# nilsbore/gp_compressor

Measured on AMD Instinct MI355X. Metric: patches/sec (compress+predict), higher is better.
Workload: dtype f64; 1 GPU; C2 room scan: 8192 patches x 256 pts per GPU, RBF + Gaussian noise, dense Cholesky fit + predictive mean on the 20x20 grid (m=400); patches_per_gpu=8192, points_per_patch=256, grid_points=400, parallelism=1 GPU, kernel=dense_mfma_w1

## Files before the change

gp_compressor_amd/csrc/dense_mfma_w1.hip:

```cpp
#include <cstdio>
#include <cstdlib>
#include <type_traits>

#include "gpc_device.h"
#include "dense_internal.h"
#include "mfma_tile.h"

#define W1_NPAD_MAX 512
#define W1_C 4
#define W1_NDT 10
#define W1_NT_OF(npad) ((npad) / 16)
#define W1_TRI_OF(npad) (W1_NT_OF(npad) * (W1_NT_OF(npad) + 1) / 2)
#define W1_TILE(i, j) (((size_t)(i) * (size_t)((i) + 1) / 2 + (size_t)(j)) * MF_IMG)
#define W1_PACK_OF(npad) ((npad) <= 256)
#define W1_LNV_OF(npad) (W1_PACK_OF(npad) ? W1_NT_OF(npad) / 2 : W1_NT_OF(npad))


struct W1Params {
    DenseArgs a;
    double c_exp;
    double pivot_tol;
    double cs, noise_u, sfp, a_out;
    double* ws;
    double* linvt;
    int export_factor;
    unsigned long long* stamps;
};
#define W1_NPH 12
#ifdef W1_STAMPS
#define W1_STAMP(ph)                                                                                                 \
    do {                                                                                                             \
        __builtin_amdgcn_sched_barrier(0);                                                                           \
        const unsigned long long t_now_ = __builtin_amdgcn_s_memtime();                                              \
        st_acc_[ph] += t_now_ - t_prev_;                                                                             \
        t_prev_ = t_now_;                                                                                            \
        __builtin_amdgcn_sched_barrier(0);                                                                           \
    } while (0)
#else
#define W1_STAMP(ph) do { } while (0)
#endif

#define W1_LDS_SYNC()                                                                                                \
    do {                                                                                                             \
        __builtin_amdgcn_fence(__ATOMIC_SEQ_CST, "wavefront");                                                       \
        __builtin_amdgcn_wave_barrier();                                                                             \
    } while (0)

template <int A, int B, typename F>
__device__ static __forceinline__ void w1_static_for(F&& f)
{
    if constexpr (A < B) {
        f(std::integral_constant<int, A>{});
        w1_static_for<A + 1, B>(f);
    }
}
__host__ __device__ constexpr int w1_stream_col(int q)
{
    int kk = 0;
    while ((kk + 1) * (kk + 2) / 2 <= q) ++kk;
    return kk;
}
__host__ __device__ constexpr int w1_pstream_pair(int q)
{
    int pp = 0;
    while (2 * (pp + 1) * (pp + 1) <= q) ++pp;
    return pp;
}
#define W1_BW 20

__device__ static __forceinline__ d4 w1_mfma4_neg(d4 a, d4 b, d4 acc)
{
#pragma unroll
    for (int s = 0; s < 4; ++s) acc = __builtin_amdgcn_mfma_f64_16x16x4f64(a[s], b[s], acc, 0, 0, 1);
    return acc;
}
__device__ static __forceinline__ d4 w1_trsm(d4 lv, d4 src)
{
    const d4 z4 = d4{0.0, 0.0, 0.0, 0.0};
    d4 D = __builtin_amdgcn_mfma_f64_16x16x4f64(lv[0], src[0], z4, 0, 0, 0);
    D = __builtin_amdgcn_mfma_f64_16x16x4f64(lv[1], src[1], D, 0, 0, 0);
    D = __builtin_amdgcn_mfma_f64_16x16x4f64(lv[2], src[2], D, 0, 0, 0);
    return __builtin_amdgcn_mfma_f64_16x16x4f64(lv[3], src[3], D, 0, 0, 0);
}

template <int MODE, int CNT, bool DIAG>
__device__ static __forceinline__ void w1_gram_row(d4 (&v)[W1_C], const double* px0, const double* px1, const double* T, double sf, bool scale_sf,
                                                   double cexp, double noise, bool dbl, int n, int r, int c0, int lr, int lg)
{
    const int pi = MF_TS * r + lr;
    const double xi0 = px0[pi], xi1 = px1[pi];
#pragma unroll
    for (int t = 0; t < CNT; ++t) {
#pragma unroll
        for (int q = 0; q < 4; ++q) {
            const int pj = MF_TS * (c0 + t) + lg + 4 * q;
            const double d0 = xi0 - px0[pj], d1 = xi1 - px1[pj];
            const double sq = __builtin_fma(d0, d0, d1 * d1);
            v[t][q] = MODE == 0 ? gpc_exp_neg(cexp * sq, T) : gpc_expm_poly<MODE == 1 ? 7 : 5>(sq);
        }
    }
    if (scale_sf) {
#pragma unroll
        for (int t = 0; t < CNT; ++t)
#pragma unroll
            for (int q = 0; q < 4; ++q) v[t][q] *= sf;
    }
    if constexpr (DIAG) {
#pragma unroll
        for (int q = 0; q < 4; ++q) {
            double d = v[CNT - 1][q] + noise;
            if (dbl) d += noise;
            v[CNT - 1][q] = (lr == lg + 4 * q) ? d : v[CNT - 1][q];
        }
    }
    if (MF_TS * (r + 1) > n || MF_TS * (c0 + CNT) > n) {
#pragma unroll
        for (int t = 0; t < CNT; ++t) {
#pragma unroll
            for (int q = 0; q < 4; ++q) {
                const int pj = MF_TS * (c0 + t) + lg + 4 * q;
                if (pi >= n || pj >= n) v[t][q] = (pi == pj) ? 1.0 : 0.0;
            }
        }
    }
}

template <int W1_NPAD>
__global__ __launch_bounds__(64, 2) void dense_w1_kernel(W1Params g)
{
    constexpr int W1_NT = W1_NT_OF(W1_NPAD), W1_TRI = W1_TRI_OF(W1_NPAD);
    __shared__ __attribute__((aligned(16))) double T[GPC_EXP_TABLE_SIZE];
    __shared__ __attribute__((aligned(16))) double px0[W1_NPAD], px1[W1_NPAD], zv[W1_NPAD];
    __shared__ __attribute__((aligned(16))) double rsbuf[32], wsc[32];
    __shared__ __attribute__((aligned(16))) double LinvC[W1_C * MF_IMG];
    constexpr bool W1_PACK = W1_PACK_OF(W1_NPAD);
    constexpr int W1_LNV = W1_LNV_OF(W1_NPAD);
    __shared__ __attribute__((aligned(16))) double dgl[W1_PACK ? W1_LNV * MF_TS : 2];

    const DenseArgs& A = g.a;
    int lane = threadIdx.x;
    int lr = lane & 15, lg = lane >> 4;
#define W1_FRESH_LANE()                                                                                              \
    do {                                                                                                             \
        lane = mf_opaque(lane);                                                                                      \
        lr = lane & 15;                                                                                              \
        lg = lane >> 4;                                                                                              \
    } while (0)
    const int m = A.m;
    const double sf = A.prm.sigmaf_sq, cexp = g.c_exp;
    const bool dbl = A.prm.ref_double_noise != 0;
    const int patch = blockIdx.x;
    double* Lt = g.ws + (size_t)patch * W1_TRI * MF_IMG;
    double* LinvTg = g.linvt + (size_t)patch * W1_LNV * MF_IMG;

    gpc_exp_table_init(T);
    {
        const int o = __builtin_amdgcn_readfirstlane(A.off[patch]);
        const int n = __builtin_amdgcn_readfirstlane(A.off[patch + 1]) - o;
        double* fs = A.f_star + (size_t)patch * m;
        __syncthreads();
        if (n <= 0 || n > W1_NPAD) {
            for (int p = lane; p < m; p += 64) fs[p] = (n == 0) ? 0.0 : __builtin_nan("");
            if (lane == 0 && A.status) A.status[patch] = (n == 0) ? GPC_STATUS_OK : GPC_STATUS_NAN;
            return;
        }
        const int nt = __builtin_amdgcn_readfirstlane((n + MF_TS - 1) / MF_TS);
#ifdef W1_STAMPS
        unsigned long long st_acc_[W1_NPH] = {};
        unsigned long long t_prev_ = __builtin_amdgcn_s_memtime();
#endif

        const double xo0 = A.x0[o], xo1 = A.x1[o];
        double qr0[W1_NPAD / 64], qr1[W1_NPAD / 64];
        double mn0 = xo0, mx0 = xo0, mn1 = xo1, mx1 = xo1;
#pragma unroll
        for (int u = 0; u < W1_NPAD / 64; ++u) {
            const int i = lane + 64 * u;
            const bool live = i < n;
            qr0[u] = live ? A.x0[o + i] : xo0;
            qr1[u] = live ? A.x1[o + i] : xo1;
            mn0 = __builtin_fmin(mn0, qr0[u]); mx0 = __builtin_fmax(mx0, qr0[u]);
            mn1 = __builtin_fmin(mn1, qr1[u]); mx1 = __builtin_fmax(mx1, qr1[u]);
            zv[i] = live ? A.y[o + i] : 0.0;
        }
#pragma unroll
        for (int o_ = 32; o_ > 0; o_ >>= 1) {
            mn0 = __builtin_fmin(mn0, __shfl_xor(mn0, o_, 64)); mx0 = __builtin_fmax(mx0, __shfl_xor(mx0, o_, 64));
            mn1 = __builtin_fmin(mn1, __shfl_xor(mn1, o_, 64)); mx1 = __builtin_fmax(mx1, __shfl_xor(mx1, o_, 64));
        }
        int mode_g, mode_p;
        {
            const bool nan_box = !((mx0 - mn0) + (mx1 - mn1) < __builtin_inf());
            const double rx = mx0 - mn0, ry = mx1 - mn1;
            const double tg = nan_box ? __builtin_inf() : -cexp * __builtin_fma(rx, rx, ry * ry);
            const double hb = 0.5 * A.grid_res;
            const double bx = hb + __builtin_fmax(__builtin_fabs(mn0), __builtin_fabs(mx0));
            const double by = hb + __builtin_fmax(__builtin_fabs(mn1), __builtin_fabs(mx1));
            const double bq = __builtin_fmax(bx, by);
            const double tp = nan_box ? __builtin_inf() : -cexp * (bq * bq);
            mode_g = __builtin_amdgcn_readfirstlane(tg <= GPC_EXP_TINY_MAX ? 2 : tg <= GPC_EXP_SMALL_MAX ? 1 : 0);
            mode_p = __builtin_amdgcn_readfirstlane(tp <= GPC_EXP_TINY_MAX ? 2 : tp <= GPC_EXP_SMALL_MAX ? 1 : 0);
            if (mode_g == 0) mode_p = 0;
        }
        const bool scaled = mode_g > 0;
        {
            const double cs = scaled ? g.cs : 1.0;
            const double co0 = scaled ? xo0 : 0.0, co1 = scaled ? xo1 : 0.0;
#pragma unroll
            for (int u = 0; u < W1_NPAD / 64; ++u) {
                const int i = lane + 64 * u;
                const bool live = i < n;
                px0[i] = live ? cs * (qr0[u] - co0) : 0.0;
                px1[i] = live ? cs * (qr1[u] - co1) : 0.0;
            }
        }
        const bool scale_sf = g.export_factor != 0;
        const double noise_u = g.noise_u, ptol = g.pivot_tol;
        W1_LDS_SYNC();
#define W1_GRAM_ROW(v, CNT, DIAG, r, c0)                                                                              \
    do {                                                                                                             \
        if (mode_g == 2) w1_gram_row<2, CNT, DIAG>(v, px0, px1, T, sf, scale_sf, cexp, noise_u, dbl, n, r, c0, lr, lg);   \
        else if (mode_g == 1) w1_gram_row<1, CNT, DIAG>(v, px0, px1, T, sf, scale_sf, cexp, noise_u, dbl, n, r, c0, lr, lg); \
        else w1_gram_row<0, CNT, DIAG>(v, px0, px1, T, sf, scale_sf, cexp, noise_u, dbl, n, r, c0, lr, lg);            \
    } while (0)

        auto bw_close = [&](auto HASW, auto REV, const int k, const d4 img, d4& pa) __attribute__((always_inline)) {
            constexpr bool has_w = decltype(HASW)::value, rev = decltype(REV)::value;
            d4 ub = d4{0.0, 0.0, 0.0, 0.0};
            if constexpr (has_w) {
                const double tot = mf_row_reduce4(pa, lr);
                if ((lr & 3) == 0) wsc[lg + 4 * (lr >> 2)] = tot;
                W1_LDS_SYNC();
            }
            if (lr == 0) {
#pragma unroll
                for (int q4 = 0; q4 < 4; ++q4) {
                    const int e = rev ? MF_TS - 1 - (lg + 4 * q4) : lg + 4 * q4;
                    ub[q4] = has_w ? zv[MF_TS * k + e] - wsc[e] : zv[MF_TS * k + e];
                }
            }
            const d4 al = w1_trsm(img, ub);
            W1_LDS_SYNC();
            if (lr == 0) {
#pragma unroll
                for (int r = 0; r < 4; ++r) zv[MF_TS * k + (rev ? MF_TS - 1 - (lg + 4 * r) : lg + 4 * r)] = al[r];
            }
            W1_LDS_SYNC();
            pa = d4{0.0, 0.0, 0.0, 0.0};
        };
        auto bw_step = [&](auto P, const d4 img, d4& pa) __attribute__((always_inline)) {
            constexpr int q = decltype(P)::value;
            constexpr int kk = w1_stream_col(q), t = q - kk * (kk + 1) / 2;
            if (kk < nt) {
                const int k = nt - 1 - kk;
                if constexpr (t < kk) {
                    const double a_ = zv[MF_TS * (k + 1 + t) + lr];
                    pa += img * a_;
                } else {
                    bw_close(std::bool_constant<(kk > 0)>{}, std::false_type{}, k, img, pa);
                }
            }
        };
        bool bad = false;
        W1_STAMP(0);
#define W1_BLOCK_ROW(bi, kb, nb)                                                                                     \
    do {                                                                                                             \
        if ((bi) < (nb)) {                                                                                           \
            d4 gv[W1_C];                                                                                             \
            W1_GRAM_ROW(gv, (bi) + 1, true, (kb) + (bi), (kb));                                                      \
            _Pragma("unroll") for (int bc = 0; bc <= (bi); ++bc) tacc[(bi) * ((bi) + 1) / 2 + bc] = gv[bc];           \
        } else {                                                                                                     \
            _Pragma("unroll") for (int bc = 0; bc <= (bi); ++bc) tacc[(bi) * ((bi) + 1) / 2 + bc] = d4{0.0, 0.0, 0.0, 0.0}; \
        }                                                                                                            \
    } while (0)
#define W1_BLOCK_INIT(kb, nb)                                                                                        \
    do {                                                                                                             \
        _Pragma("unroll") for (int i = 0; i < W1_C; ++i) part[i] = 0.0;                                              \
                                             \
        __builtin_amdgcn_sched_barrier(0);                                                                           \
        W1_BLOCK_ROW(3, kb, nb);                                                                                     \
        __builtin_amdgcn_sched_barrier(0);                                                                           \
        W1_BLOCK_ROW(2, kb, nb);                                                                                     \
        __builtin_amdgcn_sched_barrier(0);                                                                           \
        W1_BLOCK_ROW(1, kb, nb);                                                                                     \
        __builtin_amdgcn_sched_barrier(0);                                                                           \
        W1_BLOCK_ROW(0, kb, nb);                                                                                     \
        __builtin_amdgcn_sched_barrier(0);                                                                           \
    } while (0)
        W1_STAMP(1);
        for (int k = 0;; k += W1_C) {
            const int nc = min(W1_C, nt - k);
            const int kl = k - 1;
            const bool last_step = k + W1_C >= nt;
            W1_FRESH_LANE();
            const double* rrow[W1_C];
#pragma unroll
            for (int i = 0; i < W1_C; ++i) rrow[i] = Lt + W1_TILE(k + min(i, nc - 1), 0);
            d4 tacc[W1_NDT];
            double part[W1_C];
            d4 op[2][W1_C];
#pragma unroll
            for (int i = 0; i < W1_C; ++i) op[0][i] = op[1][i] = d4{0.0, 0.0, 0.0, 0.0};
            if (k > 0) {
#pragma unroll
                for (int i = 0; i < W1_C; ++i) op[0][i] = mf_img_load(rrow[i], lane);
            }
            W1_BLOCK_INIT(k, nc);
            for (int j = 0; j < k; j += 2) {
#pragma unroll
                for (int h = 0; h < 2; ++h) {
                    const int jn = min(j + h + 1, kl);
#pragma unroll
                    for (int i = 0; i < W1_C; ++i) op[h ^ 1][i] = mf_img_load(rrow[i] + (size_t)jn * MF_IMG, lane);
#pragma unroll
                    for (int d = 0; d < W1_NDT; ++d) {
                        const int bi = d >= 6 ? 3 : d >= 3 ? 2 : d >= 1 ? 1 : 0, bc = d - bi * (bi + 1) / 2;
                        if (bi < nc) tacc[d] = w1_mfma4_neg(op[h][bc], op[h][bi], tacc[d]);
                    }
                    const double* zq = zv + MF_TS * (j + h) + lg;
                    const double z0 = zq[0], z1 = zq[4], z2 = zq[8], z3 = zq[12];
#pragma unroll
                    for (int c = 0; c < W1_C; ++c) part[c] += (op[h][c][0] * z0 + op[h][c][1] * z1) + (op[h][c][2] * z2 + op[h][c][3] * z3);
                }
            }
            W1_STAMP(2);
            W1_FRESH_LANE();
            d4 Lb[W1_C * (W1_C - 1) / 2];
#pragma unroll
            for (int q = 0; q < W1_C * (W1_C - 1) / 2; ++q) Lb[q] = d4{0.0, 0.0, 0.0, 0.0};
            bool ok = mf_diag_factor_c(tacc[0], rsbuf, LinvC, W1_PACK ? nullptr : LinvTg + (size_t)k * MF_IMG, ptol, lane);
            W1_LDS_SYNC();
            if (g.export_factor) mf_img_store(Lt + W1_TILE(k, k), lane, mf_img_load(LinvC, lane));
#pragma unroll
            for (int i = 1; i < W1_C; ++i) {
                if (ok && i < nc) {
#pragma unroll
                    for (int c = 0; c < i; ++c) {
                        d4 Tt = tacc[i * (i + 1) / 2 + c];
#pragma unroll
                        for (int c2 = 0; c2 < c; ++c2) Tt = w1_mfma4_neg(Lb[c * (c - 1) / 2 + c2], Lb[i * (i - 1) / 2 + c2], Tt);
                        const d4 lvc = mf_img_load(LinvC + c * MF_IMG, mf_opaque(lane));
                        const d4 L = w1_trsm(lvc, Tt);
                        Lb[i * (i - 1) / 2 + c] = L;
                        mf_img_store(Lt + W1_TILE(k + i, k + c), lane, L);
                    }
                    d4 Dii = tacc[i * (i + 1) / 2 + i];
#pragma unroll
                    for (int c = 0; c < i; ++c) Dii = w1_mfma4_neg(Lb[i * (i - 1) / 2 + c], Lb[i * (i - 1) / 2 + c], Dii);
                    ok = mf_diag_factor_c(Dii, rsbuf, LinvC + i * MF_IMG, W1_PACK ? nullptr : LinvTg + (size_t)(k + i) * MF_IMG, ptol, lane);
                    W1_LDS_SYNC();
                    if (g.export_factor) mf_img_store(Lt + W1_TILE(k + i, k + i), lane, mf_img_load(LinvC + i * MF_IMG, mf_opaque(lane)));
                }
            }
            if (!ok) { bad = true; break; }
            if constexpr (W1_PACK) {
                if (!last_step) {
#pragma unroll
                    for (int h = 0; h < 2; ++h) {
                        const int lp = mf_opaque(lane), pr = (k >> 1) + h;
                        const double* Lo = LinvC + (2 * h + 1) * MF_IMG;
                        const d4 pk = mf_tri_pack(mf_img_load_t(LinvC + 2 * h * MF_IMG, lp), mf_img_load_tr(Lo, lp));
                        mf_img_store(LinvTg + (size_t)pr * MF_IMG, lp, pk);
                        if (lp < MF_TS) dgl[MF_TS * pr + lp] = Lo[mf_img_rc(MF_TS - 1 - lp, MF_TS - 1 - lp)];
                    }
                }
            }
            W1_STAMP(3);
            W1_FRESH_LANE();
#pragma unroll
            for (int c = 0; c < W1_C; ++c) {
                if (c < nc) {
                    const int pj = MF_TS * (k + c) + lr;
                    double pp = part[c];
#pragma unroll
                    for (int c2 = 0; c2 < c; ++c2) {
                        const d4 lb = Lb[c * (c - 1) / 2 + c2];
                        const double* zq = zv + MF_TS * (k + c2) + lg;
                        pp += (lb[0] * zq[0] + lb[1] * zq[4]) + (lb[2] * zq[8] + lb[3] * zq[12]);
                    }
                    pp += __shfl_xor(pp, 16, 64);
                    pp += __shfl_xor(pp, 32, 64);
                    const double yv = zv[pj];
                    W1_LDS_SYNC();
                    if (lg == 0) zv[pj] = yv - pp;
                    W1_LDS_SYNC();
                    const d4 lv = mf_img_load(LinvC + c * MF_IMG, mf_opaque(lane));
                    const double* tq = zv + MF_TS * (k + c) + lg;
                    double zz = (lv[0] * tq[0] + lv[1] * tq[4]) + (lv[2] * tq[8] + lv[3] * tq[12]);
                    zz += __shfl_xor(zz, 16, 64);
                    zz += __shfl_xor(zz, 32, 64);
                    W1_LDS_SYNC();
                    if (lg == 0) zv[pj] = zz;
                    W1_LDS_SYNC();
                }
            }
            W1_STAMP(4);
            const int rows_tot = nt - (k + nc);
            if (rows_tot == 0) {
                __syncthreads();
                break;
            }
            if (k > 0) __syncthreads();
            const int npass = (rows_tot + 3) / 4;
            const int klp = k - 1;
            if (k == 0) {
                for (int pi_ = 0; pi_ < npass; ++pi_) {
                    const int first_row0 = (pi_ + 1 < npass) ? 4 * (pi_ + 1) : 0;
                    const int np4 = min(4, rows_tot - first_row0);
                    W1_FRESH_LANE();
                    d4 cy[W1_C][4];
#pragma unroll
                    for (int t = 0; t < 4; ++t) {
                        const int r_ = W1_C + first_row0 + min(t, np4 - 1);
                        d4 gv[W1_C];
                        W1_GRAM_ROW(gv, 2, false, r_, 0);
                        cy[0][t] = gv[0]; cy[1][t] = gv[1];
                        __builtin_amdgcn_sched_barrier(0);
                        W1_GRAM_ROW(gv, 2, false, r_, 2);
                        cy[2][t] = gv[0]; cy[3][t] = gv[1];
                        __builtin_amdgcn_sched_barrier(0);
                    }
                    W1_STAMP(5);
#pragma unroll
                    for (int c = 0; c < W1_C; ++c) {
                        const d4 lv = mf_img_load(LinvC + c * MF_IMG, mf_opaque(lane));
#pragma unroll
                        for (int t = 0; t < 4; ++t) {
#pragma unroll
                            for (int c2 = 0; c2 < c; ++c2) cy[c][t] = w1_mfma4_neg(Lb[c * (c - 1) / 2 + c2], cy[c2][t], cy[c][t]);
                            cy[c][t] = w1_trsm(lv, cy[c][t]);
                            if (t < np4) mf_img_store(Lt + W1_TILE(W1_C + first_row0 + t, c), lane, cy[c][t]);
                        }
                    }
                    W1_STAMP(7);
                }
            }
            if (k > 0) {
                for (int pi_ = 0; pi_ < npass; ++pi_) {
                    const int first_row = (pi_ + 1 < npass) ? 4 * (pi_ + 1) : 0;
                    const int np4 = min(4, rows_tot - first_row);
                    W1_FRESH_LANE();
                    d4 cy[W1_C][4];
                    int rr[4];
                    const double* rw_[4];
#pragma unroll
                    for (int t = 0; t < 4; ++t) {
                        rr[t] = k + W1_C + first_row + min(t, np4 - 1);
                        rw_[t] = Lt + W1_TILE(rr[t], 0);
                    }
                    d4 A2[2][W1_C], B[4];
#pragma unroll
                    for (int c = 0; c < W1_C; ++c) A2[0][c] = mf_img_load(rrow[c], lane);
#pragma unroll
                    for (int t = 0; t < 4; ++t) B[t] = mf_img_load(rw_[t], lane);
#pragma unroll
                    for (int t = 0; t < 4; ++t) {
                        d4 gv[W1_C];
                        W1_GRAM_ROW(gv, 2, false, rr[t], k);
                        cy[0][t] = gv[0]; cy[1][t] = gv[1];
                        __builtin_amdgcn_sched_barrier(0);
                        W1_GRAM_ROW(gv, 2, false, rr[t], k + 2);
                        cy[2][t] = gv[0]; cy[3][t] = gv[1];
                        __builtin_amdgcn_sched_barrier(0);
                    }
                    W1_STAMP(5);
                    d4 Lq[W1_C * (W1_C - 1) / 2];
#define W1_PASS_J(st, jn, PREFETCH)                                                                                  \
    do {                                                                                                             \
                                      \
        if (PREFETCH) {                                                                                              \
            _Pragma("unroll") for (int c = 0; c < W1_C; ++c) A2[(st) ^ 1][c] = mf_img_load(rrow[c] + (size_t)(jn) * MF_IMG, lane); \
        }                                                                                                            \
        __builtin_amdgcn_sched_barrier(0);                                                                           \
        _Pragma("unroll") for (int t = 0; t < 4; ++t) {                                                              \
            _Pragma("unroll") for (int c = 0; c < W1_C; ++c) cy[c][t] = w1_mfma4_neg(A2[st][c], B[t], cy[c][t]);      \
            __builtin_amdgcn_sched_barrier(0);                                                                       \
            if (PREFETCH) B[t] = mf_img_load(rw_[t] + (size_t)(jn) * MF_IMG, lane);                                    \
            else {      \
                if (t < 3) Lq[t] = mf_img_load(Lt + W1_TILE(k + (t == 0 ? 1 : 2), k + (t == 2 ? 1 : 0)), lane);      \
                else {                                                                                               \
                    _Pragma("unroll") for (int c2 = 0; c2 < 3; ++c2) Lq[3 + c2] = mf_img_load(Lt + W1_TILE(k + 3, k + c2), lane); \
                }                                                                                                    \
            }                                                                                                        \
            __builtin_amdgcn_sched_barrier(0);                                                                       \
        }                                                                                                            \
    } while (0)
                    for (int j = 0; j + 2 < k; j += 2) {
                        W1_PASS_J(0, j + 1, true);
                        W1_PASS_J(1, j + 2, true);
                    }
                    W1_PASS_J(0, klp, true);
                    W1_PASS_J(1, klp, false);
#undef W1_PASS_J
                    W1_STAMP(6);
                    W1_FRESH_LANE();
#pragma unroll
                    for (int c = 0; c < W1_C; ++c) {
                        const d4 lv = mf_img_load(LinvC + c * MF_IMG, mf_opaque(lane));
#pragma unroll
                        for (int t = 0; t < 4; ++t) {
#pragma unroll
                            for (int c2 = 0; c2 < c; ++c2) cy[c][t] = w1_mfma4_neg(Lq[c * (c - 1) / 2 + c2], cy[c2][t], cy[c][t]);
                            cy[c][t] = w1_trsm(lv, cy[c][t]);
                            if (t < np4) mf_img_store(Lt + W1_TILE(rr[t], k + c), lane, cy[c][t]);
                        }
                    }
                    W1_STAMP(7);
                }
            }
            __syncthreads();
            W1_STAMP(8);
        }
#undef W1_BLOCK_INIT
#undef W1_BLOCK_ROW

        if (bad) {
            for (int p = lane; p < m; p += 64) fs[p] = __builtin_nan("");
            if (A.alpha_out)
                for (int i = lane; i < n; i += 64) A.alpha_out[o + i] = __builtin_nan("");
            if (lane == 0 && A.status) A.status[patch] = GPC_STATUS_NOT_SPD;
            return;
        }

        if constexpr (W1_PACK) {
            W1_FRESH_LANE();
            constexpr int NP = W1_NT;
            constexpr int SLEN = NP * NP / 2;
            const int nte = (nt + 1) & ~1, kls = (nt - 1) & ~(W1_C - 1);
            d4 win[W1_BW];
            auto stream_addr = [&](auto P) __attribute__((always_inline)) -> const double* {
                constexpr int q = decltype(P)::value;
                constexpr int pp = w1_pstream_pair(q), i = q - 2 * pp * pp;
                if constexpr (i == 2 * pp) {
                    const int k = nte - 1 - 2 * pp;
                    return (k >= 1 && k - 1 < kls) ? LinvTg + (size_t)(k >> 1) * MF_IMG : Lt;
                } else {
                    constexpr int kk = i < 2 * pp ? 2 * pp : 2 * pp + 1, t = i < 2 * pp ? i : i - 2 * pp - 1;
                    const int k = nte - 1 - kk, kq = max(k, 0);
                    return (k >= 0 && k + 1 + t < nt) ? Lt + W1_TILE(kq + 1 + t, kq) : Lt;
                }
            };
            w1_static_for<0, W1_BW>([&](auto P) __attribute__((always_inline)) {
                constexpr int q = decltype(P)::value;
                win[q] = mf_img_load_nt(stream_addr(P), lane);
            });
            d4 pa = d4{0.0, 0.0, 0.0, 0.0};
            double* const held = LinvC + (W1_C - 1) * MF_IMG;
            w1_static_for<0, SLEN>([&](auto P) __attribute__((always_inline)) {
                constexpr int q = decltype(P)::value;
                constexpr int pp = w1_pstream_pair(q), i = q - 2 * pp * pp;
                const d4 img = win[q % W1_BW];
                if constexpr (i == 2 * pp) {
                    const int k = nte - 1 - 2 * pp;
                    if (k >= 1) {
                        d4 lo;
                        bool in_lds = false;
                        if constexpr (pp < W1_C / 2) in_lds = k - 1 >= kls;
                        if (in_lds) {
                            const double* Lc = LinvC + (k - 1 - kls) * MF_IMG;
                            lo = mf_img_load_tr(Lc + MF_IMG, lane);
                        } else {
                            mf_img_store(held, lane, mf_tri_upper(img));
                            lo = mf_tri_lower(img, dgl[MF_TS * (k >> 1) + lr]);
                            W1_LDS_SYNC();
                        }
                        if (k < nt) bw_close(std::bool_constant<(pp > 0)>{}, std::true_type{}, k, lo, pa);
                    }
                } else {
                    constexpr int kk = i < 2 * pp ? 2 * pp : 2 * pp + 1, t = i < 2 * pp ? i : i - 2 * pp - 1;
                    const int k = nte - 1 - kk;
                    if (k >= 0 && k + 1 + t < nt) {
                        const double a_ = zv[MF_TS * (k + 1 + t) + lr];
                        pa += img * a_;
                    }
                    if constexpr (i == 4 * pp + 1) {
                        if (k >= 0) {
                            bool in_lds = false;
                            if constexpr (pp < W1_C / 2) in_lds = k >= kls;
                            const d4 up = in_lds ? mf_img_load_t(LinvC + (k - kls) * MF_IMG, lane) : mf_img_load(held, lane);
                            bw_close(std::true_type{}, std::false_type{}, k, up, pa);
                        }
                    }
                }
                if constexpr (q + W1_BW < SLEN) {
                    win[q % W1_BW] = mf_img_load_nt(stream_addr(std::integral_constant<int, q + W1_BW>{}), lane);
                }
            });
        } else {
            W1_FRESH_LANE();
            constexpr int NP = W1_NPAD / MF_TS;
            constexpr int SLEN = NP * (NP + 1) / 2;
            d4 win[W1_BW];
            auto stream_addr = [&](auto P) __attribute__((always_inline)) -> const double* {
                constexpr int q = decltype(P)::value;
                constexpr int kk = w1_stream_col(q), t = q - kk * (kk + 1) / 2;
                const int kq = max(nt - 1 - kk, 0);
                const double* ad = (t < kk) ? Lt + W1_TILE(kq + 1 + t, kq) : LinvTg + (size_t)kq * MF_IMG;
                return kk < nt ? ad : Lt;
            };
            w1_static_for<0, W1_BW>([&](auto P) __attribute__((always_inline)) {
                constexpr int q = decltype(P)::value;
                win[q] = mf_img_load_nt(stream_addr(P), lane);
            });
            d4 pa = d4{0.0, 0.0, 0.0, 0.0};
            w1_static_for<0, SLEN>([&](auto P) __attribute__((always_inline)) {
                constexpr int q = decltype(P)::value;
                bw_step(P, win[q % W1_BW], pa);
                if constexpr (q + W1_BW < SLEN) {
                    win[q % W1_BW] = mf_img_load_nt(stream_addr(std::integral_constant<int, q + W1_BW>{}), lane);
                }
            });
        }
        W1_STAMP(9);
        double* av = zv;
        if (A.alpha_out)
            for (int i = lane; i < n; i += 64) A.alpha_out[o + i] = av[i] * g.a_out;

        W1_FRESH_LANE();
        if (m <= 0) {
        } else if (A.xs0 == nullptr && A.grid_sz <= 32) {
            const int sz = A.grid_sz;
            const double res = A.grid_res;
            d4 P[2][2];
#pragma unroll
            for (int mt = 0; mt < 2; ++mt)
#pragma unroll
                for (int nl = 0; nl < 2; ++nl) P[mt][nl] = d4{0.0, 0.0, 0.0, 0.0};
            double gqx[2], gqy[2];
            const double cs = scaled ? g.cs : 1.0, co0 = scaled ? A.x0[o] : 0.0, co1 = scaled ? A.x1[o] : 0.0;
            const double argc = scaled ? -1.0 : cexp, sfp = g.sfp;
#pragma unroll
            for (int h = 0; h < 2; ++h) {
                const double gq = res * (((double)(16 * h + lr) + 0.5) / (double)sz - 0.5);
                gqx[h] = cs * (gq - co0);
                gqy[h] = cs * (gq - co1);
            }
            auto predict_loop = [&](auto mode_tag) __attribute__((always_inline)) {
                constexpr int MP = decltype(mode_tag)::value;
                for (int ibase = 0; ibase < n; ibase += 32) {
#pragma unroll
                    for (int s = 0; s < 8; ++s) {
                        const int i = ibase + 4 * s + lg;
                        const int ic = min(i, W1_NPAD - 1);
                        const double al = (i < n) ? sfp * av[ic] : 0.0;
                        const double xi0 = px0[ic], xi1 = px1[ic];
                        double ea[2], eb[2];
#pragma unroll
                        for (int h = 0; h < 2; ++h) {
                            const double dy = gqy[h] - xi1, dx = gqx[h] - xi0;
                            if constexpr (MP == 0) {
                                ea[h] = gpc_exp_neg(argc * (dy * dy), T);
                                eb[h] = gpc_exp_neg(argc * (dx * dx), T) * al;
                            } else {
                                ea[h] = gpc_expm_poly<MP == 1 ? 7 : 5>(dy * dy);
                                eb[h] = gpc_expm_poly<MP == 1 ? 7 : 5>(dx * dx) * al;
                            }
                        }
#pragma unroll
                        for (int nl = 0; nl < 2; ++nl)
#pragma unroll
                            for (int mt = 0; mt < 2; ++mt)
                                P[mt][nl] = __builtin_amdgcn_mfma_f64_16x16x4f64(ea[mt], eb[nl], P[mt][nl], 0, 0, 0);
                    }
                }
            };
            if (mode_p == 2) predict_loop(std::integral_constant<int, 2>{});
            else if (mode_p == 1) predict_loop(std::integral_constant<int, 1>{});
            else predict_loop(std::integral_constant<int, 0>{});
#pragma unroll
            for (int mt = 0; mt < 2; ++mt)
#pragma unroll
                for (int nl = 0; nl < 2; ++nl)
#pragma unroll
                    for (int r = 0; r < 4; ++r) {
                        const int py = 16 * mt + lg + 4 * r, pxx = 16 * nl + lr;
                        if (py < sz && pxx < sz) fs[py * sz + pxx] = P[mt][nl][r];
                    }
        } else {
            const double cs = scaled ? g.cs : 1.0, co0 = scaled ? A.x0[o] : 0.0, co1 = scaled ? A.x1[o] : 0.0;
            const double argc = scaled ? -1.0 : cexp, sfp = g.sfp;
            for (int p = lane; p < m; p += 64) {
                double q0, q1;
                if (A.xs0) {
                    q0 = A.xs0[p];
                    q1 = A.xs1[p];
                } else {
                    const int gx = p % A.grid_sz, gy = p / A.grid_sz;
                    q0 = A.grid_res * (((double)gx + 0.5) / (double)A.grid_sz - 0.5);
                    q1 = A.grid_res * (((double)gy + 0.5) / (double)A.grid_sz - 0.5);
                }
                q0 = cs * (q0 - co0);
                q1 = cs * (q1 - co1);
                double s_ = 0.0;
                for (int i = 0; i < n; ++i) {
                    const double d0 = px0[i] - q0, d1 = px1[i] - q1;
                    s_ += gpc_exp_neg(argc * __builtin_fma(d0, d0, d1 * d1), T) * av[i];
                }
                fs[p] = sfp * s_;
            }
        }
        if (lane == 0 && A.status) A.status[patch] = GPC_STATUS_OK;
#ifdef W1_STAMPS
        W1_STAMP(10);
        if (g.stamps && lane == 0)
            for (int q_ = 0; q_ < W1_NPH; ++q_) atomicAdd(g.stamps + q_, st_acc_[q_]);
#endif
    }
}

static int w1_npad(const DenseArgs& a) { return a.n_max <= 256 ? 256 : W1_NPAD_MAX; }

bool dense_w1_supported(const DenseArgs& a)
{
    if (a.v_star) return a.n_max <= 256 && a.ny == 1 && !a.sel && a.xs0 != nullptr;
    return a.n_max <= W1_NPAD_MAX && a.ny == 1 && !a.sel;
}

#define W1_MAX_SLOTS 8192
static int w1_chunk(const DenseArgs& a, int cap_in)
{
    const char* e = getenv("GPC_W1_SLOTS");
    int cap = e && atoi(e) > 0 ? atoi(e) : W1_MAX_SLOTS;
    if (cap_in > 0 && cap_in < cap) cap = cap_in;
    return a.P < cap ? a.P : cap;
}

size_t dense_w1_ws_bytes(const gpc_ctx* ctx, const DenseArgs& a, int* grid_out, int cap)
{
    (void)ctx;
    const int grid = w1_chunk(a, cap);
    if (grid_out) *grid_out = grid;
    const int npad = w1_npad(a);
    return sizeof(double) * ((size_t)(W1_TRI_OF(npad) + W1_LNV_OF(npad)) * MF_IMG * (size_t)grid + (a.v_star ? (size_t)a.n_total : 0));
}

int dense_w1_launch(gpc_ctx* ctx, const DenseSite& site, const DenseArgs& a_in, int grid)
{
    DenseArgs a = a_in;
    double* v_star = a.v_star;
    a.v_star = nullptr;
    W1Params g;
    g.c_exp = (double)(-0.5f) / a.prm.l_sq;
    g.ws = reinterpret_cast<double*>(dense_ws(ctx, site));
    const int npad = w1_npad(a);
    g.linvt = g.ws + (size_t)W1_TRI_OF(npad) * MF_IMG * (size_t)grid;
    g.export_factor = v_star ? 1 : 0;
    const double sf = a.prm.sigmaf_sq;
    const bool unit = !v_star;
    g.cs = sqrt(-g.c_exp);
    g.noise_u = unit ? a.prm.noise / sf : a.prm.noise;
    g.pivot_tol = GPC_PIVOT_RTOL * (unit ? 1.0 + a.prm.noise / sf : sf + a.prm.noise);
    g.sfp = unit ? 1.0 : sf;
    g.a_out = unit ? 1.0 / sf : 1.0;
    g.stamps = nullptr;
    if (v_star) {
        a.m = 0;
        if (!a.alpha_out) a.alpha_out = g.linvt + (size_t)W1_LNV_OF(npad) * MF_IMG * (size_t)grid;
    }
    ctx->last_dense_kernel = v_star ? "dense_mfma_w1 + dense_variance" : npad == 256 ? "dense_mfma_w1" : "dense_mfma_w1_512";
#ifdef W1_STAMPS
    if (getenv("GPC_W1_STAMPS")) {
        GPC_HIP(ctx, hipMalloc(&g.stamps, sizeof(unsigned long long) * W1_NPH));
        GPC_HIP(ctx, hipMemsetAsync(g.stamps, 0, sizeof(unsigned long long) * W1_NPH, site.stream));
    }
#endif
    for (int base = 0; base < a.P; base += grid) {
        const int cnt = a.P - base < grid ? a.P - base : grid;
        g.a = a;
        g.a.P = cnt;
        g.a.off = a.off + base;
        g.a.f_star = a.f_star ? a.f_star + (size_t)base * a.ny * a_in.m : nullptr;
        g.a.status = a.status ? a.status + base : nullptr;
        if (npad == 256) hipLaunchKernelGGL((dense_w1_kernel<256>), dim3(cnt), dim3(64), 0, site.stream, g);
        else hipLaunchKernelGGL((dense_w1_kernel<W1_NPAD_MAX>), dim3(cnt), dim3(64), 0, site.stream, g);
        GPC_HIP(ctx, hipGetLastError());
        if (v_star) {
            DenseArgs av = g.a;
            av.m = a_in.m;
            const int rc = dense_variance_launch(ctx, site, av, W1_NT_OF(256), g.ws, a.alpha_out, v_star + (size_t)base * a_in.m);
            if (rc != GPC_OK) return rc;
        }
    }
#ifdef W1_STAMPS
    if (g.stamps) {
        unsigned long long h[W1_NPH];
        GPC_HIP(ctx, hipStreamSynchronize(site.stream));
        GPC_HIP(ctx, hipMemcpy(h, g.stamps, sizeof(h), hipMemcpyDeviceToHost));
        (void)hipFree(g.stamps);
        static const char* names[W1_NPH] = {"load", "sweep gram", "sweep loop", "chain", "forward", "pass gram", "pass loop", "pass trsm",
                                            "step fence", "backward", "predict", ""};
        unsigned long long tot = 0;
        for (int q = 0; q < W1_NPH; ++q) tot += h[q];
        fprintf(stderr, "[GPC_W1_STAMPS] mean s_memtime ticks per patch (total %.0f)\n", (double)tot / a.P);
        for (int q = 0; q < 11; ++q) fprintf(stderr, "  %-12s %9.0f  %5.1f %%\n", names[q], (double)h[q] / a.P, 100.0 * h[q] / tot);
    }
#endif
    return GPC_OK;
}
```

gp_compressor_amd/csrc/mfma_tile.h:

```cpp
#pragma once

#include "gpc_device.h"

typedef double d4 __attribute__((ext_vector_type(4)));
#define MF_TS 16

__device__ static __forceinline__ int mf_opaque(int v)
{
    asm volatile("" : "+v"(v));
    return v;
}

__device__ static __forceinline__ bool mf_wait_ge(unsigned lds_byte_addr, int k)
{
    int v, cnt;
    asm volatile(
        "s_mov_b32 %1, 0x100000\n\t"
        "1:\n\t"
        "ds_read_b32 %0, %2\n\t"
        "s_waitcnt lgkmcnt(0)\n\t"
        "v_cmp_gt_i32 vcc, %3, %0\n\t"
        "s_cbranch_vccz 2f\n\t"
        "s_sub_u32 %1, %1, 1\n\t"
        "s_cmp_eq_u32 %1, 0\n\t"
        "s_cbranch_scc1 2f\n\t"
        "s_sleep 1\n\t"
        "s_branch 1b\n\t"
        "2:\n\t"
        : "=&v"(v), "=&s"(cnt)
        : "v"(lds_byte_addr), "v"(k)
        : "vcc", "scc", "memory");
    return cnt != 0;
}
__device__ static __forceinline__ void mf_publish(int* word, int k)
{
    __hip_atomic_store(word, k, __ATOMIC_RELEASE, __HIP_MEMORY_SCOPE_WORKGROUP);
}

__device__ static __forceinline__ double mf_readlane(double v, int lane_const)
{
    const int lo = __builtin_amdgcn_readlane(__double2loint(v), lane_const);
    const int hi = __builtin_amdgcn_readlane(__double2hiint(v), lane_const);
    return __hiloint2double(hi, lo);
}

__device__ static __forceinline__ double mf_rsqrt(double d)
{
    double y = __builtin_amdgcn_rsq(d);
    double e = __builtin_fma(-d * y, y, 1.0);
    y = __builtin_fma(y * 0.5, e, y);
    e = __builtin_fma(-d * y, y, 1.0);
    y = __builtin_fma(y * 0.5, e, y);
    return y;
}
__device__ static __forceinline__ double mf_rcp(double d)
{
    double y = __builtin_amdgcn_rcp(d);
    double e = __builtin_fma(-d, y, 1.0);
    y = __builtin_fma(y, e, y);
    e = __builtin_fma(-d, y, 1.0);
    y = __builtin_fma(y, e, y);
    return y;
}

typedef double d2 __attribute__((ext_vector_type(2)));
#define MF_IMG 256
__device__ static __forceinline__ int mf_img_off(int l, int s) { return (s >> 1) * 128 + l * 2 + (s & 1); }
__device__ static __forceinline__ int mf_img_rc(int r, int c) { return mf_img_off(r + 16 * (c & 3), c >> 2); }
__device__ static __forceinline__ d4 mf_img_load(const double* img, int l)
{
    const d2 a = *reinterpret_cast<const d2*>(img + l * 2);
    const d2 b = *reinterpret_cast<const d2*>(img + 128 + l * 2);
    return d4{a[0], a[1], b[0], b[1]};
}
__device__ static __forceinline__ void mf_img_store(double* img, int l, d4 v)
{
    *reinterpret_cast<d2*>(img + l * 2) = d2{v[0], v[1]};
    *reinterpret_cast<d2*>(img + 128 + l * 2) = d2{v[2], v[3]};
}

__device__ static __forceinline__ d4 mf_img_load_nt(const double* img, int l)
{
    const d2 a = __builtin_nontemporal_load(reinterpret_cast<const d2*>(img + l * 2));
    const d2 b = __builtin_nontemporal_load(reinterpret_cast<const d2*>(img + 128 + l * 2));
    return d4{a[0], a[1], b[0], b[1]};
}
__device__ static __forceinline__ void mf_img_store_nt(double* img, int l, d4 v)
{
    __builtin_nontemporal_store(d2{v[0], v[1]}, reinterpret_cast<d2*>(img + l * 2));
    __builtin_nontemporal_store(d2{v[2], v[3]}, reinterpret_cast<d2*>(img + 128 + l * 2));
}

template <bool OPAQUE = false>
__device__ __forceinline__ static bool mf_diag_factor(d4 W, double* rsbuf, double* Linv_out, double* LinvT_out, double pivot_tol, int lane_in = -1)
{
    const int lane = OPAQUE ? mf_opaque(lane_in >= 0 ? lane_in : (int)(threadIdx.x & 63)) : (int)(threadIdx.x & 63);
    const int lr = lane & 15, lg = lane >> 4;
    double rp = mf_rcp(mf_readlane(W[0], 0));
    double rpv = (lg == 0 && lr > 0) ? rp : 0.0;
    double one_q = (lg == 0) ? 1.0 : 0.0, ev = (lane == 0) ? 1.0 : 0.0;
#pragma unroll
    for (int c = 0; c < MF_TS - 1; ++c) {
        const int q = c & 3, r = c >> 2, q1 = (c + 1) & 3, r1 = (c + 1) >> 2;
        if constexpr (!OPAQUE) {
            one_q = (lg == q) ? 1.0 : 0.0;
            ev = (lg == q && lr == c) ? 1.0 : 0.0;
        }
        const double a_op = W[r] * rpv;
        const double b_op = __builtin_fma(W[r], one_q, ev);
        const d4 Wn = __builtin_amdgcn_mfma_f64_16x16x4f64(a_op, b_op, W, 0, 0, 1);
        __builtin_amdgcn_sched_barrier(0);
        const double s01 = mf_readlane(W[r], 16 * q + c + 1);
        const double s11 = mf_readlane(W[r1], 16 * q1 + c + 1);
        const double t = s01 * rp;
        rp = mf_rcp(__builtin_fma(-t, s01, s11));
        if constexpr (OPAQUE) {
            const int lo_ = mf_opaque(lane);
            const int lr_ = lo_ & 15, lg_ = lo_ >> 4;
            rpv = (lg_ == q1 && lr_ > c + 1) ? rp : 0.0;
            one_q = (lg_ == q1) ? 1.0 : 0.0;
            ev = (lo_ == 16 * q1 + c + 1) ? 1.0 : 0.0;
        } else {
            rpv = (lg == q1 && lr > c + 1) ? rp : 0.0;
        }
        __builtin_amdgcn_sched_barrier(0);
        W = Wn;
    }
    const int lt_ = OPAQUE ? mf_opaque(lane) : lane;
    const int lrt = lt_ & 15, lgt = lt_ >> 4;
    const int rsel = lrt >> 2;
    const double pd = rsel == 0 ? W[0] : rsel == 1 ? W[1] : rsel == 2 ? W[2] : W[3];
    const bool on_diag = (lrt & 3) == lgt;
    const bool ok = __builtin_amdgcn_ballot_w64(on_diag && !(pd > pivot_tol)) == 0;
    const double rs = mf_rsqrt(on_diag ? pd : 1.0);
    if (on_diag) rsbuf[lrt] = rs;
    d4 fin;
#pragma unroll
    for (int r = 0; r < 4; ++r) {
        const int row = lgt + 4 * r;
        const double rsr = rsbuf[row];
        fin[r] = (lrt < row) ? W[r] * rsr : (lrt == row ? rsr : 0.0);
    }
    mf_img_store(LinvT_out, lt_, fin);
#pragma unroll
    for (int r = 0; r < 4; ++r) Linv_out[mf_img_rc(lgt + 4 * r, lrt)] = fin[r];
    return ok;
}

__device__ static __forceinline__ int mf_sel32(int v, unsigned long long mask)
{
    int r;
    asm("v_cndmask_b32_e64 %0, 0, %1, %2" : "=v"(r) : "v"(v), "s"(mask));
    return r;
}
__device__ static __forceinline__ double mf_sel64(double v, unsigned long long mask)
{
    return __hiloint2double(mf_sel32(__double2hiint(v), mask), mf_sel32(__double2loint(v), mask));
}
__device__ static __forceinline__ double mf_one_in(unsigned long long mask, int one_hi)
{
    return __hiloint2double(mf_sel32(one_hi, mask), 0);
}
__device__ __forceinline__ static bool mf_diag_factor_c(d4 W, double* rsbuf, double* Linv_out, double* LinvT_out, double pivot_tol, int lane_in)
{
    const int one_hi = 0x3FF00000;
    double rp = mf_rcp(mf_readlane(W[0], 0));
    double rpv = mf_sel64(rp, 0xFFFEull);
    double one_q = mf_one_in(0xFFFFull, one_hi);
    double ev = mf_one_in(0x1ull, one_hi);
#pragma unroll
    for (int c = 0; c < MF_TS - 1; ++c) {
        const int q = c & 3, r = c >> 2, q1 = (c + 1) & 3, r1 = (c + 1) >> 2;
        const double a_op = W[r] * rpv;
        const double b_op = __builtin_fma(W[r], one_q, ev);
        const d4 Wn = __builtin_amdgcn_mfma_f64_16x16x4f64(a_op, b_op, W, 0, 0, 1);
        __builtin_amdgcn_sched_barrier(0);
        const double s01 = mf_readlane(W[r], 16 * q + c + 1);
        const double s11 = mf_readlane(W[r1], 16 * q1 + c + 1);
        const double t = s01 * rp;
        rp = mf_rcp(__builtin_fma(-t, s01, s11));
        const unsigned long long slot = 0xFFFFull << (16 * q1);
        const unsigned long long below = ((0xFFFFull << (c + 2)) & 0xFFFFull) << (16 * q1);
        rpv = mf_sel64(rp, below);
        one_q = mf_one_in(slot, one_hi);
        ev = mf_one_in(1ull << (16 * q1 + c + 1), one_hi);
        __builtin_amdgcn_sched_barrier(0);
        W = Wn;
    }
    const int lt_ = mf_opaque(lane_in);
    const int lrt = lt_ & 15, lgt = lt_ >> 4;
    const int rsel = lrt >> 2;
    const double pd = rsel == 0 ? W[0] : rsel == 1 ? W[1] : rsel == 2 ? W[2] : W[3];
    const bool on_diag = (lrt & 3) == lgt;
    const bool ok = __builtin_amdgcn_ballot_w64(on_diag && !(pd > pivot_tol)) == 0;
    const double rs = mf_rsqrt(on_diag ? pd : 1.0);
    if (on_diag) rsbuf[lrt] = rs;
    d4 fin;
#pragma unroll
    for (int r = 0; r < 4; ++r) {
        const int row = lgt + 4 * r;
        const double rsr = rsbuf[row];
        fin[r] = (lrt < row) ? W[r] * rsr : (lrt == row ? rsr : 0.0);
    }
    if (LinvT_out) mf_img_store(LinvT_out, lt_, fin);
#pragma unroll
    for (int r = 0; r < 4; ++r) Linv_out[mf_img_rc(lgt + 4 * r, lrt)] = fin[r];
    return ok;
}

__host__ __device__ constexpr unsigned long long mf_tri_mask(int s, int kind)
{
    unsigned long long m = 0;
    for (int l = 0; l < 64; ++l) {
        const int r = l & 15, c = (l >> 4) + 4 * s;
        if (kind == 0 ? r <= c : kind == 1 ? r == c : r > c) m |= 1ull << l;
    }
    return m;
}
__device__ static __forceinline__ int mf_mix32(int a, int b, unsigned long long mask)
{
    int r;
    asm("v_cndmask_b32_e64 %0, %1, %2, %3" : "=v"(r) : "v"(b), "v"(a), "s"(mask));
    return r;
}
__device__ static __forceinline__ double mf_mix64(double a, double b, unsigned long long mask)
{
    return __hiloint2double(mf_mix32(__double2hiint(a), __double2hiint(b), mask), mf_mix32(__double2loint(a), __double2loint(b), mask));
}
__device__ static __forceinline__ d4 mf_tri_pack(d4 up, d4 lo)
{
    constexpr unsigned long long u0 = mf_tri_mask(0, 0), u1 = mf_tri_mask(1, 0), u2 = mf_tri_mask(2, 0), u3 = mf_tri_mask(3, 0);
    return d4{mf_mix64(up[0], lo[0], u0), mf_mix64(up[1], lo[1], u1), mf_mix64(up[2], lo[2], u2), mf_mix64(up[3], lo[3], u3)};
}
__device__ static __forceinline__ d4 mf_tri_upper(d4 p)
{
    constexpr unsigned long long u0 = mf_tri_mask(0, 0), u1 = mf_tri_mask(1, 0), u2 = mf_tri_mask(2, 0), u3 = mf_tri_mask(3, 0);
    return d4{mf_sel64(p[0], u0), mf_sel64(p[1], u1), mf_sel64(p[2], u2), mf_sel64(p[3], u3)};
}
__device__ static __forceinline__ d4 mf_tri_lower(d4 p, double dg)
{
    constexpr unsigned long long l0 = mf_tri_mask(0, 2), l1 = mf_tri_mask(1, 2), l2 = mf_tri_mask(2, 2), l3 = mf_tri_mask(3, 2);
    constexpr unsigned long long e0 = mf_tri_mask(0, 1), e1 = mf_tri_mask(1, 1), e2 = mf_tri_mask(2, 1), e3 = mf_tri_mask(3, 1);
    return d4{mf_mix64(dg, mf_sel64(p[0], l0), e0), mf_mix64(dg, mf_sel64(p[1], l1), e1), mf_mix64(dg, mf_sel64(p[2], l2), e2),
              mf_mix64(dg, mf_sel64(p[3], l3), e3)};
}
__device__ static __forceinline__ d4 mf_img_load_t(const double* img, int l)
{
    const int lr = l & 15, lg = l >> 4;
    return d4{img[mf_img_rc(lg, lr)], img[mf_img_rc(lg + 4, lr)], img[mf_img_rc(lg + 8, lr)], img[mf_img_rc(lg + 12, lr)]};
}
__device__ static __forceinline__ d4 mf_img_load_tr(const double* img, int l)
{
    const int lr = 15 - (l & 15), lg = 15 - (l >> 4);
    return d4{img[mf_img_rc(lg, lr)], img[mf_img_rc(lg - 4, lr)], img[mf_img_rc(lg - 8, lr)], img[mf_img_rc(lg - 12, lr)]};
}

__device__ static __forceinline__ double mf_row_dot(const double* img, int mr, const double* v)
{
    double s_ = 0.0;
#pragma unroll
    for (int gq = 0; gq < 4; ++gq) {
        const d4 ch = mf_img_load(img, mr + 16 * gq);
#pragma unroll
        for (int s = 0; s < 4; ++s) s_ = __builtin_fma(ch[s], v[gq + 4 * s], s_);
    }
    return s_;
}

template <int CTRL>
__device__ static __forceinline__ double mf_dpp(double v)
{
    const int lo = __builtin_amdgcn_mov_dpp(__double2loint(v), CTRL, 0xf, 0xf, true);
    const int hi = __builtin_amdgcn_mov_dpp(__double2hiint(v), CTRL, 0xf, 0xf, true);
    return __hiloint2double(hi, lo);
}
__device__ static __forceinline__ double mf_row_allsum(double v)
{
    v += mf_dpp<0x121>(v);
    v += mf_dpp<0x122>(v);
    v += mf_dpp<0x124>(v);
    v += mf_dpp<0x128>(v);
    return v;
}

__device__ static __forceinline__ double mf_row_reduce4(d4 x, int lr)
{
    const bool hi8 = (lr & 8) != 0, hi4 = (lr & 4) != 0;
    double k0 = hi8 ? x[2] : x[0], k1 = hi8 ? x[3] : x[1];
    const double s0 = hi8 ? x[0] : x[2], s1 = hi8 ? x[1] : x[3];
    k0 += mf_dpp<0x128>(s0);
    k1 += mf_dpp<0x128>(s1);
    double k = hi4 ? k1 : k0;
    const double sd = hi4 ? k0 : k1;
    k += mf_dpp<0x141>(sd);
    k += mf_dpp<0xB1>(k);
    k += mf_dpp<0x4E>(k);
    return k;
}
```

Baseline: 5.624 million patches/s.

## Reverse panel traversal order for cache reuse and pin select masks in SGPRs

The Cholesky panel update loop now walks prior tile columns from most recent to oldest, and the trailing-row update passes alternate between ascending and descending j order. This serpentine traversal is meant to reuse factor tiles still resident in cache from the previous pass. Select and mix masks are also materialised through explicit s_mov_b32 literals so the compiler keeps them in scalar registers instead of rematerialising them. The reordering changes the floating-point summation order of the accumulation, and the volatile asm may constrain scheduling.

Measured after the change: 5.608 million patches/s. No clear change (-0.3%).

```diff
diff --git a/gp_compressor_amd/csrc/dense_mfma_w1.hip b/gp_compressor_amd/csrc/dense_mfma_w1.hip
--- a/gp_compressor_amd/csrc/dense_mfma_w1.hip
+++ b/gp_compressor_amd/csrc/dense_mfma_w1.hip
@@ -303,13 +303,14 @@
             for (int i = 0; i < W1_C; ++i) op[0][i] = op[1][i] = d4{0.0, 0.0, 0.0, 0.0};
             if (k > 0) {
 #pragma unroll
-                for (int i = 0; i < W1_C; ++i) op[0][i] = mf_img_load(rrow[i], lane);
+                for (int i = 0; i < W1_C; ++i) op[0][i] = mf_img_load(rrow[i] + (size_t)kl * MF_IMG, lane);
             }
             W1_BLOCK_INIT(k, nc);
             for (int j = 0; j < k; j += 2) {
 #pragma unroll
                 for (int h = 0; h < 2; ++h) {
-                    const int jn = min(j + h + 1, kl);
+                    const int jc = kl - (j + h);
+                    const int jn = max(jc - 1, 0);
 #pragma unroll
                     for (int i = 0; i < W1_C; ++i) op[h ^ 1][i] = mf_img_load(rrow[i] + (size_t)jn * MF_IMG, lane);
 #pragma unroll
@@ -317,7 +318,7 @@
                         const int bi = d >= 6 ? 3 : d >= 3 ? 2 : d >= 1 ? 1 : 0, bc = d - bi * (bi + 1) / 2;
                         if (bi < nc) tacc[d] = w1_mfma4_neg(op[h][bc], op[h][bi], tacc[d]);
                     }
-                    const double* zq = zv + MF_TS * (j + h) + lg;
+                    const double* zq = zv + MF_TS * jc + lg;
                     const double z0 = zq[0], z1 = zq[4], z2 = zq[8], z3 = zq[12];
 #pragma unroll
                     for (int c = 0; c < W1_C; ++c) part[c] += (op[h][c][0] * z0 + op[h][c][1] * z1) + (op[h][c][2] * z2 + op[h][c][3] * z3);
@@ -449,10 +450,12 @@
                         rw_[t] = Lt + W1_TILE(rr[t], 0);
                     }
                     d4 A2[2][W1_C], B[4];
-#pragma unroll
-                    for (int c = 0; c < W1_C; ++c) A2[0][c] = mf_img_load(rrow[c], lane);
-#pragma unroll
-                    for (int t = 0; t < 4; ++t) B[t] = mf_img_load(rw_[t], lane);
+                    const bool desc = (pi_ & 1) != 0;
+#define W1_JMAP(x) (desc ? klp - (x) : (x))
+#pragma unroll
+                    for (int c = 0; c < W1_C; ++c) A2[0][c] = mf_img_load(rrow[c] + (size_t)W1_JMAP(0) * MF_IMG, lane);
+#pragma unroll
+                    for (int t = 0; t < 4; ++t) B[t] = mf_img_load(rw_[t] + (size_t)W1_JMAP(0) * MF_IMG, lane);
 #pragma unroll
                     for (int t = 0; t < 4; ++t) {
                         d4 gv[W1_C];
@@ -486,12 +489,13 @@
         }                                                                                                            \
     } while (0)
                     for (int j = 0; j + 2 < k; j += 2) {
-                        W1_PASS_J(0, j + 1, true);
-                        W1_PASS_J(1, j + 2, true);
-                    }
-                    W1_PASS_J(0, klp, true);
+                        W1_PASS_J(0, W1_JMAP(j + 1), true);
+                        W1_PASS_J(1, W1_JMAP(j + 2), true);
+                    }
+                    W1_PASS_J(0, W1_JMAP(klp), true);
                     W1_PASS_J(1, klp, false);
 #undef W1_PASS_J
+#undef W1_JMAP
                     W1_STAMP(6);
                     W1_FRESH_LANE();
 #pragma unroll
diff --git a/gp_compressor_amd/csrc/mfma_tile.h b/gp_compressor_amd/csrc/mfma_tile.h
--- a/gp_compressor_amd/csrc/mfma_tile.h
+++ b/gp_compressor_amd/csrc/mfma_tile.h
@@ -147,19 +147,27 @@
     return ok;
 }
 
-__device__ static __forceinline__ int mf_sel32(int v, unsigned long long mask)
+__device__ static __forceinline__ unsigned long long mf_lit64(unsigned long long mask)
+{
+    unsigned lo, hi;
+    asm volatile("s_mov_b32 %0, %1" : "=s"(lo) : "i"((unsigned)mask));
+    asm volatile("s_mov_b32 %0, %1" : "=s"(hi) : "i"((unsigned)(mask >> 32)));
+    return ((unsigned long long)hi << 32) | lo;
+}
+__device__ static __forceinline__ int mf_sel32_s(int v, unsigned long long smask)
 {
     int r;
-    asm("v_cndmask_b32_e64 %0, 0, %1, %2" : "=v"(r) : "v"(v), "s"(mask));
+    asm("v_cndmask_b32_e64 %0, 0, %1, %2" : "=v"(r) : "v"(v), "s"(smask));
     return r;
 }
 __device__ static __forceinline__ double mf_sel64(double v, unsigned long long mask)
 {
-    return __hiloint2double(mf_sel32(__double2hiint(v), mask), mf_sel32(__double2loint(v), mask));
+    const unsigned long long sm = mf_lit64(mask);
+    return __hiloint2double(mf_sel32_s(__double2hiint(v), sm), mf_sel32_s(__double2loint(v), sm));
 }
 __device__ static __forceinline__ double mf_one_in(unsigned long long mask, int one_hi)
 {
-    return __hiloint2double(mf_sel32(one_hi, mask), 0);
+    return __hiloint2double(mf_sel32_s(one_hi, mf_lit64(mask)), 0);
 }
 __device__ __forceinline__ static bool mf_diag_factor_c(d4 W, double* rsbuf, double* Linv_out, double* LinvT_out, double pivot_tol, int lane_in)
 {
@@ -225,7 +233,8 @@
 }
 __device__ static __forceinline__ double mf_mix64(double a, double b, unsigned long long mask)
 {
-    return __hiloint2double(mf_mix32(__double2hiint(a), __double2hiint(b), mask), mf_mix32(__double2loint(a), __double2loint(b), mask));
+    const unsigned long long sm = mf_lit64(mask);
+    return __hiloint2double(mf_mix32(__double2hiint(a), __double2hiint(b), sm), mf_mix32(__double2loint(a), __double2loint(b), sm));
 }
 __device__ static __forceinline__ d4 mf_tri_pack(d4 up, d4 lo)
 {
```
